# JeremyCJM/DiffSHEG

Measured on AMD Instinct MI355X. Metric: motion frames/sec (ddim25, n_poses=88), higher is better.
Workload: dtype bf16

## Files before the change

diffsheg_amd/_lib.py:

```python
from __future__ import annotations

import ctypes as C
import os

_HERE = os.path.dirname(os.path.abspath(__file__))
LIB_PATH = os.path.join(_HERE, "libdiffsheg_hip.so")


class DshError(RuntimeError):
    pass


class ModelConfigC(C.Structure):
    _fields_ = [("dim_pose", C.c_int32), ("expression_dim", C.c_int32), ("style_dim", C.c_int32),
                ("classifier_free", C.c_int32), ("cond_scale", C.c_float), ("latent_dim", C.c_int32),
                ("ff_size", C.c_int32), ("num_layers", C.c_int32), ("num_heads", C.c_int32),
                ("audio_dim", C.c_int32), ("aud_latent_dim", C.c_int32), ("hubert_dim", C.c_int32),
                ("hubert_enc_dim", C.c_int32), ("precision", C.c_int32), ("single_transformer", C.c_int32)]


class CrossAttnWeightsC(C.Structure):
    _fields_ = [(n, C.c_void_p) for n in ("norm_g", "norm_b", "text_norm_g", "text_norm_b", "wq", "bq", "wk", "bk", "wv", "bv",
                                           "sty_norm_g", "sty_norm_b", "sty_emb_w", "sty_emb_b", "sty_out_w", "sty_out_b")]

# ... 38 lines not shown
    "dsh_sample_num_steps_from": (C.c_int64, [C.POINTER(SamplerOptsC), C.c_int32, C.c_int32, C.c_int32]),
    "dsh_invert": (C.c_int, [_P, C.POINTER(SamplerOptsC), _P, C.c_int32, _P]),
    "dsh_invert_from": (C.c_int, [_P, C.POINTER(SamplerOptsC), _P, C.c_int32, C.c_int32, _P]),
    "dsh_set_guidance_scale": (C.c_int, [_P, C.POINTER(C.c_float), C.c_int32]),
    "dsh_diffusion_table": (C.c_int32, [C.c_int32, C.c_int32, C.c_char_p, C.POINTER(C.c_double), C.c_int32]),
    "dsh_timestep_map": (C.c_int32, [C.c_int32, C.c_int32, C.POINTER(C.c_int32), C.c_int32]),
    "dsh_jump_schedule": (C.c_int32, [C.c_int32, C.c_int32, C.c_int32, C.POINTER(C.c_int32), C.c_int32]),
    "dsh_interp_time": (C.c_int, [_P, _P, C.c_int32, C.c_int32, C.c_int32, _P, C.c_int32]),
    "dsh_interp_time_ragged": (C.c_int, [_P, _P, C.c_int32, C.c_int32, C.c_int32, _P, C.c_int32, _P, _P]),
    "dsh_inv_standardize": (C.c_int, [_P, _P, C.c_int64, C.c_int32, _P, _P, _P]),
    "dsh_axis_angle_to_euler": (C.c_int, [_P, _P, C.c_int64, C.c_int64, C.c_int32, _P, _P, _P, _P, _P, C.c_int64, _P, C.c_int64, _P, C.c_int32]),
    "dsh_euler_to_axis_angle": (C.c_int, [_P, _P, C.c_int64, C.c_int64, C.c_int32, _P, _P, _P, _P, _P, C.c_int64, _P, C.c_int32]),
    "dsh_op_gemm": (C.c_int, [_P, C.c_int32, _P, _P, _P, _P, _P, _P, C.c_int32, C.c_int32, C.c_int32, C.c_int32]),
    "dsh_op_gemm_f32_pro": (C.c_int, [_P, C.c_int32] + [_P, C.c_int32, C.c_int32] * 4 + [C.c_int32, _P, _P, _P, _P, C.c_int32, C.c_int32, C.c_int32, C.c_int32, _P, _P, C.c_int32, C.c_int32, C.c_int32, _P, C.c_int32, _P]),
    "dsh_debug_last_tl_variant": (C.c_int32, []),
    "dsh_debug_launch_counts": (C.c_int32, [C.POINTER(C.c_int64), C.c_int32, C.c_int32]),
    "dsh_op_tl_linear": (C.c_int, [_P, C.c_int32, _P, _P, _P, _P, _P, _P, C.c_int32, C.c_int32, C.c_int32, _P, _P, _P, C.c_int32, C.c_int32, C.c_int32]),
    "dsh_op_tl2_ffn": (C.c_int, [_P] * 12 + [C.c_int32, C.c_int32, _P, C.c_int32, _P, _P, C.c_int32]),
    "dsh_op_tl_aud_tail": (C.c_int, [_P] * 16 + [C.c_int32, C.c_int32, C.c_int32, _P, _P, C.c_int32]),
    "dsh_op_tl_aproj": (C.c_int, [_P, _P, _P, _P, C.c_int32, _P, _P, C.c_int32]),
    "dsh_op_tl_joint": (C.c_int, [_P, _P, C.c_int32, C.c_int32, C.c_int32, _P, _P, _P, C.c_int32, _P, C.c_int32, C.c_int32, _P]),
    "dsh_op_cross_attention": (C.c_int, [_P, C.POINTER(CrossAttnWeightsC), _P, _P, _P] + [C.c_int32] * 7 + [_P]),
    "dsh_op_linear_attention": (C.c_int, [_P, _P, C.c_int32, C.c_int32, C.c_int32, C.c_int32, _P]),
    "dsh_op_linear_attention_bf16": (C.c_int, [_P, _P, C.c_int32, C.c_int32, C.c_int32, C.c_int32, _P]),
    "dsh_op_linear_attention_ragged": (C.c_int, [_P, C.c_int32, C.c_int32, _P, C.c_int32, C.c_int32, C.c_int32, C.c_int32, _P, _P, C.c_int32, _P]),
    "dsh_op_linear_attention_tiled": (C.c_int, [_P, _P, C.c_int32, C.c_int32, C.c_int32, C.c_int32, _P, _P, C.c_int32, C.c_int32]),
    "dsh_op_layernorm": (C.c_int, [_P, _P, C.c_int32, C.c_int32, _P, _P, _P]),
    "dsh_op_ddim_step": (C.c_int, [_P] * 6 + [C.c_int32] * 3 + [C.c_float] * 4 + [C.c_int32] * 6),
    "dsh_op_philox_randn": (C.c_int, [_P, _P, C.c_int64, C.c_uint64, C.c_uint64]),
    "dsh_op_q_sample": (C.c_int, [_P] * 6 + [C.c_int32] * 6 + [C.c_uint64, C.c_uint64, C.POINTER(C.c_uint64), _P, C.POINTER(C.c_int32), C.c_uint64]),
# ... 101 lines not shown
```

diffsheg_amd/csrc/capi.hip:

```cpp
#include <algorithm>
#include <cmath>
#include <cstdio>
#include <cstdlib>
#include <cstring>
#include <map>
#include <memory>
#include <vector>

#include "../../include/diffsheg_hip.h"
#include "denoiser.h"
#include "audio_front.h"
#include "fgd.h"
#include "hubert.h"
#include "sampler.h"

namespace dsh {
static thread_local std::string g_last_error;
void set_last_error(const std::string& msg) { g_last_error = msg; }
const char* last_error_cstr() { return g_last_error.c_str(); }
}

struct dsh_ctx {
    dsh::ModelConfig cfg;
    hipStream_t stream = nullptr;
// ... 369 lines not shown
    dsh::GemmProArgs a{};
    a.pro = pro;
    a.seg[0] = x0; a.seg[1] = w1 ? x1 : nullptr; a.seg[2] = w2 ? x2 : nullptr; a.seg[3] = w3 ? x3 : nullptr;
    a.seg_ld[0] = ld0; a.seg_ld[1] = ld1; a.seg_ld[2] = ld2; a.seg_ld[3] = ld3;
    a.seg_end[0] = w0 / 32; a.seg_end[1] = a.seg_end[0] + w1 / 32; a.seg_end[2] = a.seg_end[1] + w2 / 32; a.seg_end[3] = a.seg_end[2] + w3 / 32;
    a.K = 32 * a.seg_end[3]; a.k_real = k_real;
    a.W = W; a.ldw = a.K; a.bias = bias; a.fc = fc;
    a.film = film; a.film_ld = film_ld; a.film_off = film_off; a.frames = frames; a.bmod = nb;
    a.R = R; a.ldr = N; a.C = C; a.ldc = N; a.M = M; a.N = N; a.act = act; a.nt_n = a.nt_m = 0;
    a.stats = stats; a.stat_groups = stat_groups; a.stat_gs = stat_groups > 0 ? a.K / stat_groups : 0; a.stats_out = stats_out;
    return dsh::launch_gemm_f32_pro(a, reinterpret_cast<hipStream_t>(hip_stream));
    API_END
}

int32_t dsh_debug_last_tl_variant(void) { return dsh::g_tl_last_variant; }

int32_t dsh_debug_launch_counts(int64_t* out, int32_t cap, int32_t reset) {
    for (int i = 0; i < dsh::LC_COUNT; ++i) {
        const long long v = reset ? dsh::g_launch_counts[i].exchange(0, std::memory_order_relaxed) : dsh::g_launch_counts[i].load(std::memory_order_relaxed);
        if (out && i < cap) out[i] = (int64_t)v;
    }
    return dsh::LC_COUNT;
}

namespace {
struct OpScratch {
    std::vector<void*> p;
    ~OpScratch() { for (void* q : p) (void)hipFree(q); }
    int alloc(void** out, size_t bytes) { DSH_HIP_CHECK(hipMalloc(out, bytes)); p.push_back(*out); return 0; }
    int upload(void** out, const void* host, size_t bytes) {
// ... 1180 lines not shown
```

diffsheg_amd/csrc/dsh_kernels.h:

```cpp
#pragma once
#include "dsh_common.h"

namespace dsh {

struct ConcatSegs {
    const float* p0; int ld0, w0;
    const void* p1;  int ld1, w1;
    const void* p2;  int ld2, w2;
    const float* p3; int ld3, w3;
};

struct GemmProArgs {
    int pro;
    const float* seg[4]; int seg_ld[4];
    int seg_end[4];
    int k_real;
    const float* W; int ldw;
    const float* bias;
    const float* fc;
    const float* film; int film_ld, film_off, frames, bmod;
    const float* R; int ldr;
    float* C; int ldc;
    int M, N, K, act;
    int nt_n, nt_m;
// ... 47 lines not shown
    int tls_nb0, tls_tb1;
    int dbg;
    unsigned long long* clk;
    unsigned long long* trace;
};
int launch_tl_linear(const TlArgs& a, int pro, hipStream_t s);
bool tl_linear_film_clips_ok(int frames, int bmod);
bool tls_linear_supported(const TlArgs& a, int pro);
bool tls_film_clips_ok(int frames, int bmod);
int launch_tls_linear(const TlArgs& a, int pro, hipStream_t s);
int tl_weight_src_row(int r);
int launch_tl_permute_weight(const void* W, int N, int K, void* dst, hipStream_t s);

int launch_tl2_linear(const TlArgs& a, int pro, hipStream_t s);
extern int g_tl_last_variant;
size_t tl2_frag_index(int K, int nt, int n, int k);
struct Tl2FfnArgs {
    const void* X;
    const void* Wffn;
    const float* b1; const float* b2; const float* b3;
    const float* film; int film_ld, film_off, frames, bmod, half_row0;
    const float* R; float* Cf; void* Ct;
    const float* row_const; int n_const_rows;
    int M;
    unsigned long long* trace;
    unsigned long long* clk;
    int stag_groups, stag_sleep;
    int rev;
    const void* Rhi; const void* Rlo; void* Clo;
};
// ... 112 lines not shown
```

diffsheg_amd/csrc/switches.h:

```cpp
#pragma once
#include <algorithm>
#include <atomic>
#include <cstdint>
#include <cstdlib>
#include <cstring>
#include <mutex>
#include <string>

namespace dsh {

enum SwitchKind : int { SWK_INT = 0, SWK_FLAG = 1, SWK_STR = 2 };
enum SwitchWhen : int { SWW_PROCESS = 0, SWW_CONTEXT = 1, SWW_CALL = 2 };
enum SwitchClass : int { SWC_PRODUCT = 0, SWC_AB_EXACT = 1, SWC_AB_ROUNDOFF = 2, SWC_BENCH = 3 };

#define DSH_SWITCH_TABLE(X)                                                                                                                      \
    X(DUAL, "DSH_DUAL", INT, "3", CONTEXT, PRODUCT, "most sub-batch streams of a large batch: 0 one stream, 1 two, n at most n (1 .. 8); results identical") \
    X(DUAL_LAG, "DSH_DUAL_LAG", INT, "3", CONTEXT, PRODUCT, "stream i + 1 starts this many token-per-lane launches behind stream i; the sampler reads it again per loop (CALL)") \
    X(DUAL_ROWS, "DSH_DUAL_ROWS", INT, "21500 (fp32: 2900)", CONTEXT, PRODUCT, "token rows per sub-batch stream; overrides only when positive") \
    X(DUAL_MIN_ROWS, "DSH_DUAL_MIN_ROWS", INT, "12288 (fp32: 4096)", CONTEXT, PRODUCT, "smallest batch (token rows) split over sub-batch streams; overrides only when positive") \
    X(PIPE, "DSH_PIPE", INT, "1", CALL, AB_EXACT, "sampling loops: the two encoders on two streams, the gesture encoder one step behind; 0 in sequence") \
    X(PIPE_ROWS, "DSH_PIPE_ROWS", INT, "64499", PROCESS, PRODUCT, "token rows below which a loop runs ONE batch with two encoder streams; latched in the sampler, read afresh (CONTEXT) by the sub-batch splitter") \
    X(NO_GRAPH, "DSH_NO_GRAPH", FLAG, "unset", CALL, PRODUCT, "present (any value, 0 included): small-batch evaluations are not replayed from a hipGraph") \
    X(GRAPH_ROWS, "DSH_GRAPH_ROWS", INT, "4096", PROCESS, PRODUCT, "token rows up to which a sampling loop replays its evaluations from a hipGraph") \
    X(LEVEL_CACHE, "DSH_LEVEL_CACHE", INT, "1", CALL, AB_EXACT, "x-independent part of an evaluation once per timestep level; 0 on every step") \
    X(LEVEL_PREFETCH, "DSH_LEVEL_PREFETCH", INT, "1", CALL, AB_EXACT, "that part ahead of the loop on a side stream; 0 inline at a level's first use") \
    X(TL2, "DSH_TL2", INT, "1", CONTEXT, AB_ROUNDOFF, "token-per-lane Linears: 0 first generation, 1 LDS-DMA kernels, 2 LDS-DMA everywhere (fp32 residual); dsh_op_tl_linear reads it per CALL") \
    X(TL2_ROLL, "DSH_TL2_ROLL", INT, "1", CALL, AB_EXACT, "rolling main loop of q|k|v / feat_proj.1 / ffn.linear2; 0 the round-2 loop") \
    X(TL2_ROT, "DSH_TL2_ROT", INT, "0", CALL, AB_EXACT, "rolling launches walk the weight tiles in a per-block rotated order (measured neutral)") \
    X(TL2_KSKIP, "DSH_TL2_KSKIP", INT, "1", CALL, AB_EXACT, "feat_proj.1 skips the trailing all-zero fragments of the concat row; 0 multiplies all 64") \
    X(TL2_HL, "DSH_TL2_HL", INT, "1", CONTEXT, AB_EXACT, "LDS-DMA kernels for the two residual-carrying Linears on hi / lo planes; 0 first generation") \
    X(FFN_FUSE, "DSH_FFN_FUSE", INT, "1", CONTEXT, AB_ROUNDOFF, "FFN branch as one fused launch; 0 three launches") \
    X(FFN_V, "DSH_FFN_V", INT, "3", CONTEXT, AB_ROUNDOFF, "fused FFN kernel generation: only 2 selects tl2_ffn_kernel, anything else tl3_ffn_kernel; dsh_op_tl2_ffn and the profiler's class text read it per CALL") \
    X(FFN_PC, "DSH_FFN_PC", INT, "1", CALL, AB_EXACT, "fused FFN phase C: 0 the round-4 loop, 1 pipelined across the phase boundary, 2 also pass-B epilogues early (clamped to 0 .. 2)") \
    X(FFN_PB, "DSH_FFN_PB", INT, "1", CALL, AB_EXACT, "fused FFN last stage (& 3): bit 0 hi plane kept in registers, bit 1 pass-B residual requested early; the denoiser's profiler byte count latches it") \
    X(FFN_X_IS_HI, "DSH_FFN_X_IS_HI", INT, "0", CALL, BENCH, "dsh_op_tl2_ffn on hi / lo planes: the input IS the hi plane of the residual, as in the denoiser's layers") \
    X(FFN_REPEAT, "DSH_FFN_REPEAT", INT, "0", CALL, BENCH, "dsh_op_tl2_ffn launches its kernel this many extra times (results unchanged)") \
    X(HILO, "DSH_HILO", INT, "1 (op entries: 0)", CONTEXT, AB_ROUNDOFF, "bf16 residual stream as hi + lo planes; 0 fp32 + bf16 shadow.  The op entries read it per CALL and take unset as OFF (hilo_denoiser / hilo_op below)") \
    X(TLS, "DSH_TLS", INT, "1", CONTEXT, AB_EXACT, "window-chain batches on the 32-token-block kernels of tl_small.hip; 0 off") \
    X(TLS_ROWS, "DSH_TLS_ROWS", INT, "per instantiation", CONTEXT, AB_EXACT, "token rows per launch up to which those kernels are used; overrides only when positive") \
    X(REV, "DSH_REV", INT, "1", CONTEXT, AB_EXACT, "alternate the row order of consecutive large token-per-lane launches; 0 off") \
    X(STAGGER, "DSH_STAGGER", STR, "unset", PROCESS, AB_EXACT, "\"groups,sleep[,mask]\" (%d,%d,%d): staggered first-round block start; mask bit 0 fused FFN, 1 q|k|v, 2 the other Linears") \
    X(SPLIT_AT, "DSH_SPLIT_AT", STR, "unset", PROCESS, BENCH, "\"c1,c2,...\": explicit sub-batch boundaries (clip indices); the list is latched, the once-only warning looks at its presence per CONTEXT") \
// ... 118 lines not shown
```

diffsheg_amd/csrc/tl2.hip:

```cpp
#include <algorithm>
#include <cstdio>
#include <cstdlib>
#include <type_traits>

#include "dsh_common.h"
#include "dsh_kernels.h"
#include "tl_common.h"
#include "switches.h"

namespace dsh {

namespace {

__device__ __forceinline__ void dma_sel(int k, const char* src_lane, char* lds_wave) {
    const char* s4 = src_lane + (k >> 2) * 4096;
    char* d4 = lds_wave + (k >> 2) * 4096;
    switch (k & 3) {
        case 0: __builtin_amdgcn_global_load_lds((gptr_t)s4, (lptr_t)d4, 16, 0, 0); break;
        case 1: __builtin_amdgcn_global_load_lds((gptr_t)s4, (lptr_t)d4, 16, 1024, 0); break;
        case 2: __builtin_amdgcn_global_load_lds((gptr_t)s4, (lptr_t)d4, 16, 2048, 0); break;
        default: __builtin_amdgcn_global_load_lds((gptr_t)s4, (lptr_t)d4, 16, 3072, 0); break;
    }
}
template <int N>
// ... 423 lines not shown
                    }
                }
                asm volatile("" : "+v"(prev));
            }
            if (PROBE) { pp.stamp(3); pp.roll(); }
        }
    };
    do_tile(nt0, std::true_type{});
    for (int nt = nt0 + 1; nt < nt1; ++nt) do_tile(nt, std::false_type{});
#pragma unroll
    for (int i = 0; i < NSTORE; ++i) store_piece(nt1 - 1, prev, i);
    trace_mark(p.trace, 2);
    if (PROBE) pp.dump(p.clk, pc0, pw0);
}

constexpr int FFN_MAXCLIP = 3;
constexpr int FFN_CH = 32 * 1024;
constexpr int FFN_LDS = 4 * FFN_CH + FFN_MAXCLIP * 4096 + (1024 + 3 * 512) * 4;
constexpr int FFN_NQ = 64 + 16;

template <bool PROBE>
__global__ __launch_bounds__(256, 1) void tl2_ffn_kernel(Tl2FfnArgs p) {
    extern __shared__ __attribute__((aligned(16))) char smem[];
    PhaseProbe pp;
    const unsigned long long pc0 = PROBE ? __builtin_readcyclecounter() : 0, pw0 = PROBE ? wall_clock64() : 0;
    trace_mark(p.trace, 0);
    start_stagger(p.stag_groups, p.stag_sleep);
    const int tid = threadIdx.x, lane = tid & 63;
    const int wave = __builtin_amdgcn_readfirstlane(tid >> 6);
    const int ml = lane & 31, h = lane >> 5;
// ... 297 lines not shown
        p.clk[(size_t)blockIdx.x * 8 + 7] = ((pc_ln - pc0) & 0xffffffffull) | ((__builtin_readcyclecounter() - pc0) << 32);
}

void tl_stagger_config(int which, int* groups, int* sleep) {
    struct Cfg { int g = 0, sl = 0, mask = 7; };
    static const Cfg cfg = [] {
        Cfg c;
        if (const char* e = switch_str(SW_STAGGER)) { int a = 0, b = 0, m = 7; const int n = sscanf(e, "%d,%d,%d", &a, &b, &m); if (n >= 2) { c.g = a; c.sl = b; if (n >= 3) c.mask = m; } }
        return c;
    }();
    const bool on = cfg.g > 1 && ((cfg.mask >> which) & 1);
    *groups = on ? cfg.g : 0; *sleep = on ? cfg.sl : 0;
}

int g_tl_last_variant = -1;

int launch_tl2_linear(const TlArgs& a, int pro, hipStream_t s) {
    DSH_REQUIRE(a.M > 0 && a.N > 0 && a.N % 32 == 0, "tl2_linear: N must be a positive multiple of 32");
    DSH_REQUIRE(a.K == 512 || a.K == 1024, "tl2_linear: K must be 512 or 1024");
    DSH_REQUIRE(a.ldx == (pro == 3 ? 512 : a.K), "tl2_linear: the tiled input must be exactly K features wide");
    DSH_REQUIRE(((uintptr_t)a.X % 16) == 0 && ((uintptr_t)a.W % 16) == 0, "tl2_linear: operands must be 16-byte aligned");
    DSH_REQUIRE(!a.Cf || !a.cf_rowmajor || a.ldcf % 4 == 0, "tl2_linear: row-major output leading dim");
    DSH_REQUIRE(!(a.cf_rowmajor && (a.R || a.Ct)), "tl2_linear: the row-major fp32 output has no residual / bf16 shadow");
    DSH_REQUIRE(pro >= 0 && pro <= 3, "tl2_linear: unknown prologue");
    const int tok = a.K == 512 ? 256 : 128;
    DSH_REQUIRE(pro != 1 && pro != 3 || (a.bias && a.row_const), "tl2_linear: folded LayerNorm needs d (bias) and c (row_const) vectors");
    DSH_REQUIRE(pro != 2 || (a.film && a.frames > 0 && a.bmod > 0 && a.film_ld % 4 == 0 && a.film_off % 4 == 0),
                "tl2_linear: FiLM prologue needs the folded film table");
    DSH_REQUIRE(pro != 2 || std::min((tok - 1) / a.frames + 2, a.bmod) <= T2_MAXCLIP,
                "tl2_linear: FiLM prologue: too many clips per 256-token block (clips shorter than 29 frames need batch <= 10)");
    DSH_REQUIRE(pro != 2 || a.K == 512, "tl2_linear: FiLM prologue is instantiated for K = 512");
    DSH_REQUIRE(!a.row_const || pro == 1 || pro == 3 || (pro == 2 && a.R && a.act == ACT_NONE),
                "tl2_linear: row_const is the CFG-null constant of the StylizationBlock instantiation or the c vector of a folded LayerNorm");
    DSH_REQUIRE(pro != 3 || (a.K == 1024 && a.X1 && a.X2 && a.kreal > 896 - 1 && a.kreal <= 1024), "tl2_linear: concat prologue arguments");
    const int mblocks = ceil_div(a.M, tok), ntiles = a.N / 32;
    int tpb = ntiles;
    if (mblocks < 128) { tpb = 1; while (tpb < ntiles && mblocks * ceil_div(ntiles, tpb) > 256) ++tpb; }
    TlArgs b = a;
    b.tiles_per_block = tpb;
    b.rot = switch_int(SW_TL2_ROT) != 0 ? 1 : 0;
    tl_stagger_config(pro == 1 ? 1 : 2, &b.stag_groups, &b.stag_sleep);
    if (mblocks < 256) { b.stag_groups = 0; b.stag_sleep = 0; }
    const dim3 grid(mblocks, ceil_div(ntiles, tpb)), block(a.K == 512 ? 512 : 256);
    const int lds = 4 * T2_CHUNK + 2 * a.N * 4;
    DSH_REQUIRE(lds <= 160 * 1024, "tl2_linear: N too large for the LDS bias table");
    typedef void (*kern_t)(TlArgs);
    struct Variant { int k, pro, has_r, out, act; kern_t fn; };
#define TLV(P, R, O, A) {512, P, R, O, A, tl2_linear_kernel<512, P, (R) != 0, O, A>}
#define TLV1K(P, R, O, A) {1024, P, R, O, A, tl2_linear_kernel<1024, P, (R) != 0, O, A>}
    static const Variant variants[] = {
        TLV(1, 0, 2, ACT_NONE),
        TLV(2, 1, 3, ACT_NONE),
        TLV(0, 0, 2, ACT_GELU),
        TLV(0, 0, 2, ACT_NONE), TLV(0, 1, 3, ACT_NONE), TLV(0, 0, 2, ACT_SILU), TLV(1, 0, 1, ACT_NONE),
        TLV(2, 0, 2, ACT_NONE), TLV(0, 1, 1, ACT_NONE), TLV(0, 0, 1, ACT_NONE),
        TLV(0, 0, 4, ACT_NONE),
        TLV1K(0, 0, 2, ACT_NONE),
        TLV1K(0, 0, 2, ACT_SILU),
// ... 14 lines not shown
    kern_t fn = nullptr;
    int variant = 0;
    for (int i = 0; i < NV; ++i)
        if (variants[i].k == a.K && variants[i].pro == pro && variants[i].has_r == has_r && variants[i].out == out && variants[i].act == a.act) fn = variants[i].fn;
    if (a.clk) {
        kern_t pf = nullptr;
        if (a.K == 512 && pro == 1 && !has_r && out == 2) pf = tl2_linear_kernel<512, 1, false, 2, ACT_NONE, true>;
        if (a.K == 512 && pro == 2 && has_r && out == 3) pf = tl2_linear_kernel<512, 2, true, 3, ACT_NONE, true>;
        if (a.K == 1024 && pro == 0 && !has_r && out == 2 && a.act == ACT_NONE) pf = tl2_linear_kernel<1024, 0, false, 2, ACT_NONE, true>;
        if (pf) {
            DSH_HIP_CHECK(hipFuncSetAttribute(reinterpret_cast<const void*>(pf), hipFuncAttributeMaxDynamicSharedMemorySize, 160 * 1024));
            fn = pf;
        } else b.clk = nullptr;
    }
    DSH_REQUIRE(fn != nullptr || a.Rlo, "tl2_linear: this (prologue, residual, outputs, activation) combination is not instantiated");
    const bool roll_on = switch_int(SW_TL2_ROLL) != 0;
    if (roll_on && !has_r && out == 2 && !b.clk && tpb == ntiles && ntiles >= 2) {
        kern_t rf = nullptr;
        if (a.K == 512 && pro == 1 && a.act == ACT_NONE) rf = tl2_linear_kernel<512, 1, false, 2, ACT_NONE, false, true>;
        else if (a.K == 1024 && pro == 3 && a.act == ACT_SILU) {
            const int nz = switch_int(SW_TL2_KSKIP) == 0 ? 0 : (1024 - round_up(a.kreal, 16)) / 16;
            rf = nz >= 8 ? (kern_t)tl2_linear_kernel<1024, 3, false, 2, ACT_SILU, false, true, false, 8>
               : nz >= 1 ? (kern_t)tl2_linear_kernel<1024, 3, false, 2, ACT_SILU, false, true, false, 1> : (kern_t)tl2_linear_kernel<1024, 3, false, 2, ACT_SILU, false, true>;
        }
        else if (a.K == 1024 && pro == 0 && a.act == ACT_NONE) rf = tl2_linear_kernel<1024, 0, false, 2, ACT_NONE, false, true>;
        if (rf) {
            static const bool rattr = [] {
                bool ok = true;
                auto set = [&](kern_t f) { ok &= hipFuncSetAttribute(reinterpret_cast<const void*>(f), hipFuncAttributeMaxDynamicSharedMemorySize, 160 * 1024) == hipSuccess; };
                set(tl2_linear_kernel<512, 1, false, 2, ACT_NONE, false, true>); set(tl2_linear_kernel<1024, 3, false, 2, ACT_SILU, false, true>);
                set(tl2_linear_kernel<1024, 3, false, 2, ACT_SILU, false, true, false, 8>); set(tl2_linear_kernel<1024, 3, false, 2, ACT_SILU, false, true, false, 1>);
                set(tl2_linear_kernel<1024, 0, false, 2, ACT_NONE, false, true>);
                return ok;
            }();
            DSH_REQUIRE(rattr, "tl2_linear: hipFuncSetAttribute failed for the rolling instantiations");
            fn = rf;
            variant = 1;
        }
    }
    if (a.Rlo) {
        DSH_REQUIRE(a.R && a.Clo && a.Ct && !a.Cf && a.act == ACT_NONE && ((a.K == 512 && pro == 2) || (a.K == 1024 && pro == 0)),
                    "tl2_linear: hi / lo residual planes are instantiated for the StylizationBlock (K = 512) and feat_proj.3 (K = 1024) launches");
        kern_t hf = a.K == 512 ? (kern_t)tl2_linear_kernel<512, 2, true, 3, ACT_NONE, false, true, true> : (kern_t)tl2_linear_kernel<1024, 0, true, 3, ACT_NONE, false, true, true>;
        static const bool hattr = [] {
            return hipFuncSetAttribute(reinterpret_cast<const void*>(tl2_linear_kernel<512, 2, true, 3, ACT_NONE, false, true, true>), hipFuncAttributeMaxDynamicSharedMemorySize, 160 * 1024) == hipSuccess &&
                   hipFuncSetAttribute(reinterpret_cast<const void*>(tl2_linear_kernel<1024, 0, true, 3, ACT_NONE, false, true, true>), hipFuncAttributeMaxDynamicSharedMemorySize, 160 * 1024) == hipSuccess;
        }();
        DSH_REQUIRE(hattr, "tl2_linear: hipFuncSetAttribute failed for the hi / lo instantiations");
        b.clk = nullptr;
        fn = hf;
        variant = 2;
    }
    g_tl_last_variant = variant;
    count_launch(variant == 1 ? LC_TL2_ROLL : variant == 2 ? LC_TL2_ROLL_HL : LC_TL2_LOOP);
    hipLaunchKernelGGL(fn, grid, block, lds, s, b);
    DSH_HIP_CHECK(hipGetLastError());
    return 0;
}

bool tl2_ffn_supported(int M, int frames, int bmod) {
    return M >= 128 * 64 && std::min((TL_TOK - 1) / frames + 2, bmod) <= FFN_MAXCLIP;
}

int launch_tl2_ffn(const Tl2FfnArgs& a, hipStream_t s) {
    DSH_REQUIRE(a.M > 0 && a.X && a.Wffn && a.b1 && a.b2 && a.b3 && a.film && a.R && a.Cf && a.Ct, "tl2_ffn: null operand");
    DSH_REQUIRE(a.frames > 0 && a.bmod > 0 && a.film_ld % 4 == 0 && a.film_off % 4 == 0, "tl2_ffn: folded FiLM table");
    DSH_REQUIRE(std::min((TL_TOK - 1) / a.frames + 2, a.bmod) <= FFN_MAXCLIP, "tl2_ffn: too many clips per 128-token block");
    static bool attr = false;
// ... 21 lines not shown
```

diffsheg_amd/csrc/tl_linear.hip:

```cpp
#include <algorithm>
#include <cstdlib>

#include "dsh_common.h"
#include "dsh_kernels.h"
#include "tl_common.h"

namespace dsh {

template <int KD, int PRO, bool HAS_R, int OUT, int ACT, int ABL = 0, bool HL = false>
__global__ __launch_bounds__(256, (KD == 512 ? 2 : 1)) void tl_linear_kernel(TlArgs p) {
    static_assert(!HL || (HAS_R && OUT == 3 && ACT == ACT_NONE && ABL == 0), "hi / lo planes: the residual-carrying instantiations only");
    constexpr int TL_K = KD, NFRAG = KD / 16, NST = KD / TL_STAGE_K;
    constexpr bool HAS_C = (PRO == 2 && HAS_R && ACT == ACT_NONE);
    constexpr int LDS_W = tl_lds_bytes(KD);
    extern __shared__ __attribute__((aligned(16))) char smem[];
    const int tid = threadIdx.x, lane = tid & 63, wave = tid >> 6;
    unsigned long long clk0 = 0, rt0 = 0;
    if (p.clk) { clk0 = __builtin_readcyclecounter(); rt0 = wall_clock64(); }
    const int ml = lane & 31, h = lane >> 5;
    const int bx = tl_block_index(p.rev);
    const int tb = bx * (TL_TOK / 32) + wave;
    const int row = tb * 32 + ml;
    const int lane_off = ml * 32 + h * 16;

// ... 254 lines not shown
                }
            }
        }
    }
    if (p.clk && blockIdx.x == 0 && blockIdx.y == 0 && tid == 0) {
        p.clk[0] = __builtin_readcyclecounter() - clk0;
        p.clk[1] = wall_clock64() - rt0;
        p.clk[2] = bar_cyc;
    }
}

bool tl_linear_film_clips_ok(int frames, int bmod) { return frames > 0 && bmod > 0 && std::min((TL_TOK - 1) / frames + 2, bmod) <= TL_MAXCLIP; }

int launch_tl_linear(const TlArgs& a, int pro, hipStream_t s) {
    g_tl_last_variant = 10;
    DSH_REQUIRE(a.M > 0 && a.N > 0 && a.N % 32 == 0, "tl_linear: N must be a positive multiple of 32");
    DSH_REQUIRE(a.K == 512 || a.K == 1024, "tl_linear: K must be 512 or 1024");
    DSH_REQUIRE(a.ldx == (pro == 3 ? 512 : a.K), "tl_linear: the tiled input must be exactly K features wide");
    DSH_REQUIRE(((uintptr_t)a.X % 16) == 0 && ((uintptr_t)a.W % 16) == 0, "tl_linear: operands must be 16-byte aligned");
    DSH_REQUIRE(!a.Cf || !a.cf_rowmajor || a.ldcf % 4 == 0, "tl_linear: row-major output leading dim");
    DSH_REQUIRE(!(a.cf_rowmajor && (a.R || a.Ct)), "tl_linear: the row-major fp32 output has no residual / bf16 shadow");
    DSH_REQUIRE(pro == 0 || (a.gamma && a.beta), "tl_linear: LayerNorm prologue needs gamma/beta");
    DSH_REQUIRE(pro != 2 || (a.film && a.frames > 0 && a.bmod > 0 && a.film_ld % 4 == 0 && a.film_off % 4 == 0),
                "tl_linear: FiLM prologue needs the folded film table");
    DSH_REQUIRE(pro != 2 || tl_linear_film_clips_ok(a.frames, a.bmod),
                "tl_linear: FiLM prologue: too many clips per 128-token block (clips shorter than 26 frames need batch <= 6)");
    DSH_REQUIRE(pro != 2 || a.K == 512, "tl_linear: FiLM prologue is instantiated for K = 512");
    const int mblocks = ceil_div(a.M, TL_TOK), ntiles = a.N / 32, slots = a.K == 512 ? 512 : 256;
    int tpb = ntiles;
    if (mblocks < 256) { tpb = 1; while (tpb < ntiles && mblocks * ceil_div(ntiles, tpb) > slots) ++tpb; }
// ... 76 lines not shown
```

diffsheg_amd/csrc/tl_small.hip:

```cpp
#include "dsh_kernels.h"
#include "tl_common.h"

#include <algorithm>
#include <cstdlib>

namespace dsh {
namespace {

__device__ __forceinline__ void mfma16_lds_b(f32x16& acc, const u32x4* a, const char* lds_lane) {
    u32x4 bw[2][4];
#pragma unroll
    for (int i = 0; i < 4; ++i) bw[0][i] = *reinterpret_cast<const u32x4*>(lds_lane + i * 1024);
#pragma unroll
    for (int g = 0; g < 4; ++g) {
        if (g + 1 < 4) {
#pragma unroll
            for (int i = 0; i < 4; ++i) bw[(g + 1) & 1][i] = *reinterpret_cast<const u32x4*>(lds_lane + ((g + 1) * 4 + i) * 1024);
        }
#pragma unroll
        for (int i = 0; i < 4; ++i)
            acc = __builtin_amdgcn_mfma_f32_32x32x16_bf16(__builtin_bit_cast(bf16x8, a[g * 4 + i]), __builtin_bit_cast(bf16x8, bw[g & 1][i]), acc, 0, 0, 0);
    }
}

// ... 215 lines not shown
bool tls_film_clips_ok(int frames, int bmod) { return frames > 0 && bmod > 0 && std::min(31 / frames + 2, bmod) <= TLS_MAXCLIP; }

bool tls_linear_supported(const TlArgs& a, int pro) {
    if (a.M <= 0 || a.N <= 0 || a.N % 128 != 0 || !a.bias || !a.X || !a.W) return false;
    if (a.frames <= 0 || a.bmod <= 0) return false;
    const int Mc = a.frames * a.bmod;
    if (a.M != Mc && !(a.M > Mc && (a.M - Mc) % 32 == 0 && a.M - Mc >= Mc)) return false;
    if ((pro == 1 || pro == 3) && !a.row_const) return false;
    if (pro == 2 && !(a.film && a.film_ld % 4 == 0 && a.film_off % 4 == 0 && tls_film_clips_ok(a.frames, a.bmod))) return false;
    if (pro == 3 && !(a.X1 && a.X2 && a.kreal > 896 - 1 && a.kreal <= 1024)) return false;
    return tls_pick(a, pro) != nullptr;
}

int launch_tls_linear(const TlArgs& a, int pro, hipStream_t s) {
    g_tl_last_variant = 11;
    DSH_REQUIRE(tls_linear_supported(a, pro), "tls_linear: this launch is not covered by the window-chain kernels");
    DSH_REQUIRE(((uintptr_t)a.X % 16) == 0 && ((uintptr_t)a.W % 16) == 0, "tls_linear: operands must be 16-byte aligned");
    tls_kern_t fn = tls_pick(a, pro);
    static bool attr = false;
    if (!attr) {
        const tls_kern_t all[] = {tls_linear_kernel<512, 2, true, ACT_NONE>, tls_linear_kernel<1024, 0, true, ACT_NONE>,
                                  tls_linear_kernel<512, 1, false, ACT_NONE>, tls_linear_kernel<512, 0, false, ACT_GELU>,
                                  tls_linear_kernel<1024, 0, false, ACT_NONE>, tls_linear_kernel<1024, 3, false, ACT_SILU>};
        for (tls_kern_t k : all)
            DSH_HIP_CHECK(hipFuncSetAttribute(reinterpret_cast<const void*>(k), hipFuncAttributeMaxDynamicSharedMemorySize, 64 * 1024));
        attr = true;
    }
    TlArgs b = a;
    const int Mc = a.frames * a.bmod, nbh = ceil_div(std::min(a.M, Mc), 32);
    b.tls_nb0 = nbh;
// ... 11 lines not shown
```

include/diffsheg_hip.h:

```cpp
#ifndef DIFFSHEG_HIP_H
#define DIFFSHEG_HIP_H

#include <stdint.h>

#ifdef __cplusplus
extern "C" {
#endif

typedef struct dsh_ctx dsh_ctx;

enum { DSH_PRECISION_FP32 = 0, DSH_PRECISION_BF16 = 1 };
enum { DSH_SAMPLER_DDIM = 0, DSH_SAMPLER_DDPM = 1 };
enum { DSH_NOISE_STACK = 0, DSH_NOISE_PHILOX = 1 };

typedef struct dsh_model_config {
    int32_t dim_pose;
    int32_t expression_dim;
    int32_t style_dim;
    int32_t classifier_free;
    float   cond_scale;
    int32_t latent_dim;
    int32_t ff_size;
    int32_t num_layers;
    int32_t num_heads;
// ... 75 lines not shown
                        float* y);
int dsh_axis_angle_to_euler(void* hip_stream, const float* x, int64_t ld_x, int64_t rows, int32_t joints, const float* mean_aa,
                            const float* std_aa, const float* mean_e, const float* std_e, float* y_std, int64_t ld_std, float* y_deg,
                            int64_t ld_deg, const int32_t* lengths_dev, int32_t frames);
int dsh_euler_to_axis_angle(void* hip_stream, const float* x, int64_t ld_x, int64_t rows, int32_t joints, const float* mean_e,
                            const float* std_e, const float* mean_aa, const float* std_aa, float* y, int64_t ld_y,
                            const int32_t* lengths_dev, int32_t frames);

int dsh_op_gemm(void* hip_stream, int32_t dtype, const void* A, const void* W, const float* bias, const float* R,
                float* Cf, void* Ct, int32_t M, int32_t N, int32_t K, int32_t act);
int dsh_op_gemm_f32_pro(void* hip_stream, int32_t pro, const float* x0, int32_t ld0, int32_t w0, const float* x1, int32_t ld1, int32_t w1,
                        const float* x2, int32_t ld2, int32_t w2, const float* x3, int32_t ld3, int32_t w3, int32_t k_real, const float* W,
                        const float* bias, const float* fc, const float* film, int32_t film_ld, int32_t film_off, int32_t frames, int32_t nb,
                        const float* R, float* C, int32_t M, int32_t N, int32_t act, const float* stats, int32_t stat_groups, float* stats_out);
int32_t dsh_debug_last_tl_variant(void);
#define DSH_LAUNCH_COUNT_ENTRIES 17
int32_t dsh_debug_launch_counts(int64_t* out, int32_t cap, int32_t reset);
int dsh_op_tl_linear(void* hip_stream, int32_t pro, const void* X, const void* W, const float* bias, const float* R,
                     float* Cf, void* Ct, int32_t M, int32_t N, int32_t act, const float* gamma, const float* beta,
                     const float* film, int32_t frames, int32_t nb, int32_t K);
int dsh_op_tl2_ffn(void* hip_stream, const void* X, const float* Hres, const void* W1, const float* b1, const void* W2, const float* b2,
                   const void* W3, const float* b3, const float* gamma, const float* beta, const float* film, int32_t frames, int32_t nb,
                   const float* row_const, int32_t n_const_rows, float* Cf, void* Ct, int32_t M);
int dsh_op_tl_aud_tail(void* hip_stream, const void* Y, const float* X2, const float* ws1, const float* bs1, const float* w1, const float* b1,
                       const float* w2, const float* b2, const float* ws2, const float* bs2, const float* g1, const float* be1, const float* g2,
                       const float* be2, const float* film, int32_t frames, int32_t nb, int32_t Mc, float* out_f, void* out_b, int32_t ld_b);
int dsh_op_tl_aproj(void* hip_stream, const void* X, const float* W, const float* bias, int32_t n_enc, void* out0, void* out1, int32_t Mc);
int dsh_op_tl_joint(void* hip_stream, const float* x, int32_t ldx, int32_t c0, int32_t w, const float* Wj, const float* bias, const float* pe,
                    int32_t frames, const float* cnull, int32_t Mc, int32_t row1, float* h_out);
typedef struct dsh_cross_attn_weights {
// ... 142 lines not shown
```

Before: 157,900.

## Run q|k|v projection on 4 waves of 64 tokens each

Adds a dedicated q|k|v rolling kernel in which each wave holds two 32-token row blocks, one in VGPRs and one in AGPRs. Each LDS weight fragment then feeds two MFMAs, and the block uses 256 threads instead of 512. The aim is to halve LDS weight reads and DMA traffic per token and to interleave epilogue work for both blocks inside the MFMA stream. In exchange, register pressure is very high and fewer waves are resident for latency hiding. The new kernel becomes the default for K=512 rolling launches, and setting the roll switch to 2 restores the old path.

```diff
diff --git a/diffsheg_amd/_lib.py b/diffsheg_amd/_lib.py
--- a/diffsheg_amd/_lib.py
+++ b/diffsheg_amd/_lib.py
@@ -76,6 +76,7 @@
     "dsh_op_gemm": (C.c_int, [_P, C.c_int32, _P, _P, _P, _P, _P, _P, C.c_int32, C.c_int32, C.c_int32, C.c_int32]),
     "dsh_op_gemm_f32_pro": (C.c_int, [_P, C.c_int32] + [_P, C.c_int32, C.c_int32] * 4 + [C.c_int32, _P, _P, _P, _P, C.c_int32, C.c_int32, C.c_int32, C.c_int32, _P, _P, C.c_int32, C.c_int32, C.c_int32, _P, C.c_int32, _P]),
     "dsh_debug_last_tl_variant": (C.c_int32, []),
+    "dsh_debug_last_tl_wave_tokens": (C.c_int32, []),
     "dsh_debug_launch_counts": (C.c_int32, [C.POINTER(C.c_int64), C.c_int32, C.c_int32]),
     "dsh_op_tl_linear": (C.c_int, [_P, C.c_int32, _P, _P, _P, _P, _P, _P, C.c_int32, C.c_int32, C.c_int32, _P, _P, _P, C.c_int32, C.c_int32, C.c_int32]),
     "dsh_op_tl2_ffn": (C.c_int, [_P] * 12 + [C.c_int32, C.c_int32, _P, C.c_int32, _P, _P, C.c_int32]),
diff --git a/diffsheg_amd/csrc/capi.hip b/diffsheg_amd/csrc/capi.hip
--- a/diffsheg_amd/csrc/capi.hip
+++ b/diffsheg_amd/csrc/capi.hip
@@ -407,6 +407,7 @@
 }
 
 int32_t dsh_debug_last_tl_variant(void) { return dsh::g_tl_last_variant; }
+int32_t dsh_debug_last_tl_wave_tokens(void) { return dsh::g_tl_last_wave_tokens; }
 
 int32_t dsh_debug_launch_counts(int64_t* out, int32_t cap, int32_t reset) {
     for (int i = 0; i < dsh::LC_COUNT; ++i) {
diff --git a/diffsheg_amd/csrc/dsh_kernels.h b/diffsheg_amd/csrc/dsh_kernels.h
--- a/diffsheg_amd/csrc/dsh_kernels.h
+++ b/diffsheg_amd/csrc/dsh_kernels.h
@@ -85,6 +85,7 @@
 
 int launch_tl2_linear(const TlArgs& a, int pro, hipStream_t s);
 extern int g_tl_last_variant;
+extern int g_tl_last_wave_tokens;
 size_t tl2_frag_index(int K, int nt, int n, int k);
 struct Tl2FfnArgs {
     const void* X;
diff --git a/diffsheg_amd/csrc/switches.h b/diffsheg_amd/csrc/switches.h
--- a/diffsheg_amd/csrc/switches.h
+++ b/diffsheg_amd/csrc/switches.h
@@ -25,7 +25,7 @@
     X(LEVEL_CACHE, "DSH_LEVEL_CACHE", INT, "1", CALL, AB_EXACT, "x-independent part of an evaluation once per timestep level; 0 on every step") \
     X(LEVEL_PREFETCH, "DSH_LEVEL_PREFETCH", INT, "1", CALL, AB_EXACT, "that part ahead of the loop on a side stream; 0 inline at a level's first use") \
     X(TL2, "DSH_TL2", INT, "1", CONTEXT, AB_ROUNDOFF, "token-per-lane Linears: 0 first generation, 1 LDS-DMA kernels, 2 LDS-DMA everywhere (fp32 residual); dsh_op_tl_linear reads it per CALL") \
-    X(TL2_ROLL, "DSH_TL2_ROLL", INT, "1", CALL, AB_EXACT, "rolling main loop of q|k|v / feat_proj.1 / ffn.linear2; 0 the round-2 loop") \
+    X(TL2_ROLL, "DSH_TL2_ROLL", INT, "1", CALL, AB_EXACT, "rolling main loop of q|k|v / feat_proj.1 / ffn.linear2, q|k|v on 4 waves of 64 tokens; 2 q|k|v on 8 waves of 32 as the others; 0 the round-2 loop") \
     X(TL2_ROT, "DSH_TL2_ROT", INT, "0", CALL, AB_EXACT, "rolling launches walk the weight tiles in a per-block rotated order (measured neutral)") \
     X(TL2_KSKIP, "DSH_TL2_KSKIP", INT, "1", CALL, AB_EXACT, "feat_proj.1 skips the trailing all-zero fragments of the concat row; 0 multiplies all 64") \
     X(TL2_HL, "DSH_TL2_HL", INT, "1", CONTEXT, AB_EXACT, "LDS-DMA kernels for the two residual-carrying Linears on hi / lo planes; 0 first generation") \
diff --git a/diffsheg_amd/csrc/tl2.hip b/diffsheg_amd/csrc/tl2.hip
--- a/diffsheg_amd/csrc/tl2.hip
+++ b/diffsheg_amd/csrc/tl2.hip
@@ -461,6 +461,173 @@
     if (PROBE) pp.dump(p.clk, pc0, pw0);
 }
 
+__global__ __attribute__((amdgpu_flat_work_group_size(256, 256), amdgpu_waves_per_eu(1, 1)))
+void tl2_qkv_w64_kernel(TlArgs p) {
+    constexpr int NW = 4, NTHR = NW * 64, ND = 32 / NW, NFRAG = 32;
+    extern __shared__ __attribute__((aligned(16))) char smem[];
+    trace_mark(p.trace, 0);
+    start_stagger(p.stag_groups, p.stag_sleep);
+    const int tid = threadIdx.x, lane = tid & 63;
+    const int wave = __builtin_amdgcn_readfirstlane(tid >> 6);
+    const int ml = lane & 31, h = lane >> 5;
+    const int bx = tl_block_index(p.rev);
+    const int tb0 = bx * (2 * NW) + 2 * wave;
+    const int lane_off = ml * 32 + h * 16;
+    const int NT = p.N / 32;
+    const int nt0 = blockIdx.y * p.tiles_per_block;
+    const int nt1 = (nt0 + p.tiles_per_block) < NT ? (nt0 + p.tiles_per_block) : NT;
+    const int p0 = nt0, p1 = nt1;
+    char* wdst = smem + wave * (ND * 1024);
+    const __amdgpu_buffer_rsrc_t wrsrc = __builtin_amdgcn_make_buffer_rsrc(const_cast<void*>(p.W), 0, p.N * 512 * 2, 0x00020000);
+    const int wvoff = wave * (ND * 1024) + lane * 16;
+    const int ntl = nt1 - nt0;
+    const int rot = p.rot ? (int)((unsigned)(bx >> 3) % (unsigned)ntl) : 0;
+    auto ptile = [&](int nt) -> int { const int t = nt + rot; return t >= nt1 ? t - ntl : t; };
+    auto dma_soff = [&](int q) -> int { return ptile(q < p1 ? q : p1 - 1) * T2_CHUNK; };
+    auto dma_dst = [&](int q) -> char* { return wdst + (q & 3) * T2_CHUNK; };
+    auto issue_chunk = [&](int q) {
+#pragma unroll
+        for (int k = 0; k < ND; ++k) dma_buf(k, wrsrc, wvoff, dma_soff(q), dma_dst(q));
+    };
+    issue_chunk(p0);
+    issue_chunk(p0 + 1);
+    u32x4 fragA[NFRAG], fragB[NFRAG];
+    {
+        const char* xr = reinterpret_cast<const char*>(p.X) + (size_t)tb0 * NFRAG * 1024 + lane_off;
+#pragma unroll
+        for (int s = 0; s < NFRAG; ++s) fragA[s] = *reinterpret_cast<const u32x4*>(xr + s * 1024);
+#pragma unroll
+        for (int s = 0; s < NFRAG; ++s) fragB[s] = *reinterpret_cast<const u32x4*>(xr + (NFRAG + s) * 1024);
+    }
+    float* sbias = reinterpret_cast<float*>(smem + 4 * T2_CHUNK);
+    float* sconst = sbias + p.N;
+    for (int i = tid; i < p.N; i += NTHR) {
+        sbias[i] = p.bias[i];
+        sconst[i] = p.row_const[i];
+    }
+    float rstd[2], nmr[2];
+    {
+        float sum, sq;
+        row_moments_bf16<NFRAG>(fragA, sum, sq);
+        float mean = sum / 512.f;
+        sq = fmaxf(sq - sum * mean, 0.f);
+        rstd[0] = 1.0f / sqrtf(sq / 512.f + 1e-5f);
+        nmr[0] = -mean * rstd[0];
+        row_moments_bf16<NFRAG>(fragB, sum, sq);
+        mean = sum / 512.f;
+        sq = fmaxf(sq - sum * mean, 0.f);
+        rstd[1] = 1.0f / sqrtf(sq / 512.f + 1e-5f);
+        nmr[1] = -mean * rstd[1];
+    }
+#pragma unroll
+    for (int s = 0; s < NFRAG; ++s) {
+        asm volatile("" ::"v"(fragA[s]));
+        asm volatile("" : "+a"(fragB[s]));
+    }
+    asm volatile("s_waitcnt vmcnt(0)" ::: "memory");
+    __syncthreads();
+    issue_chunk(p0 + 2);
+    trace_mark(p.trace, 1);
+
+    char* Ctb = reinterpret_cast<char*>(p.Ct);
+    typedef __attribute__((address_space(3))) const char* lcptr_t;
+    typedef __attribute__((address_space(3))) const u32x4* lfrag_t;
+    const char* lds_lane_r = smem + lane * 16;
+    auto chunk_base = [&](int q) -> lcptr_t { lcptr_t b = (lcptr_t)lds_lane_r + (q & 3) * T2_CHUNK; asm volatile("" : "+v"(b)); return b; };
+    u32x4 aw[2][4];
+    f32x16 acc0A, acc0B, acc1A, acc1B;
+    constexpr int VMW = ND + 7;
+    auto mid_barrier = [&]() {
+        asm volatile("s_waitcnt vmcnt(%0)\n\ts_waitcnt lgkmcnt(0)" ::"n"(VMW) : "memory");
+        __builtin_amdgcn_s_barrier();
+        asm volatile("" ::: "memory");
+        __builtin_amdgcn_sched_barrier(0);
+    };
+    auto slot_reads = [&](int m, lcptr_t cur, lcptr_t nxt) {
+        auto rd = [&](int f) { aw[(f >> 2) & 1][f & 3] = *(lfrag_t)(cur + f * 1024); };
+        if (m < 24) rd(m + 4);
+        if (m >= 20 && m < 24) rd(m + 8);
+        if (m >= 28) aw[0][m - 28] = *(lfrag_t)(nxt + (m - 28) * 1024);
+    };
+    struct Epi { float v[8]; u32x4 o[2]; };
+    f32x4 d4, c4;
+    auto epi_step = [&](int ts, int nte, const f32x16& E, Epi& st, int qi, int step, auto inloop_tag) {
+        constexpr bool INLOOP = decltype(inloop_tag)::value;
+        if (step == 0) {
+            if (ts == 0) {
+                const int col = nte * 32 + 16 * (qi >> 1) + 8 * h + 4 * (qi & 1);
+                d4 = *reinterpret_cast<const f32x4*>(sbias + col);
+                c4 = *reinterpret_cast<const f32x4*>(sconst + col);
+            }
+        } else if (step <= 4) {
+            const int e = step - 1;
+            float x = E[4 * qi + e];
+            if constexpr (INLOOP) { const float ev = x; asm volatile("v_accvgpr_read_b32 %0, %1" : "=v"(x) : "a"(ev)); }
+            x = fmaf(x, rstd[ts], fmaf(nmr[ts], c4[e], d4[e]));
+            asm volatile("" : "+v"(x));
+            st.v[4 * (qi & 1) + e] = x;
+        } else if (step == 5) {
+            u32x4 o;
+            o.x = pack_bf16(st.v[0], st.v[1]); o.y = pack_bf16(st.v[2], st.v[3]);
+            o.z = pack_bf16(st.v[4], st.v[5]); o.w = pack_bf16(st.v[6], st.v[7]);
+            asm volatile("" : "+v"(o));
+            st.o[qi >> 1] = o;
+        } else {
+            const u32x4 o = st.o[qi >> 1];
+            u32x4* dst = reinterpret_cast<u32x4*>(Ctb + ((size_t)(tb0 + ts) * (2 * NT) + 2 * nte + (qi >> 1)) * 1024 + lane_off);
+            __builtin_nontemporal_store(o, dst);
+        }
+    };
+    auto epi_slot = [&](int ts, int nte, const f32x16& E, Epi& st, auto m_tag, auto inloop_tag) {
+        constexpr int m = decltype(m_tag)::value;
+        if constexpr (m == 1 || m == 7 || m == 13 || m == 19) epi_step(ts, nte, E, st, (m - 1) / 6, 0, inloop_tag);
+        if constexpr (m >= 3 && m <= 24 && (m - 3) % 6 < 4) epi_step(ts, nte, E, st, (m - 3) / 6, 1 + (m - 3) % 6, inloop_tag);
+        if constexpr (m == 13 || m == 25) epi_step(ts, nte, E, st, m == 13 ? 1 : 3, 5, inloop_tag);
+        if constexpr (m == 28 || m == 29) epi_step(ts, nte, E, st, m == 28 ? 1 : 3, 6, inloop_tag);
+    };
+    auto tile = [&](int nt, f32x16& W0, f32x16& W1, const f32x16& E0, const f32x16& E1, auto prev_tag) {
+        constexpr bool HAS_PREV = decltype(prev_tag)::value;
+        Epi st0, st1;
+        const int pprev = HAS_PREV ? ptile(nt - 1) : 0;
+        const lcptr_t cur = chunk_base(nt), nxt = chunk_base(nt + 1);
+        const int so_next = dma_soff(nt + 3);
+        char* dst_next = dma_dst(nt + 3);
+        static_for<32>([&](auto m_tag) {
+            constexpr int m = decltype(m_tag)::value;
+            const f32x16 z = {0.f, 0.f, 0.f, 0.f, 0.f, 0.f, 0.f, 0.f, 0.f, 0.f, 0.f, 0.f, 0.f, 0.f, 0.f, 0.f};
+            const bf16x8 a = __builtin_bit_cast(bf16x8, aw[(m >> 2) & 1][m & 3]);
+            W0 = __builtin_amdgcn_mfma_f32_32x32x16_bf16(a, __builtin_bit_cast(bf16x8, fragA[m]), m == 0 ? z : W0, 0, 0, 0);
+            if ((m & 3) == 1) dma_buf(m >> 2, wrsrc, wvoff, so_next, dst_next);
+            if (HAS_PREV) epi_slot(0, pprev, E0, st0, m_tag, std::true_type{});
+            __builtin_amdgcn_sched_barrier(0);
+            W1 = __builtin_amdgcn_mfma_f32_32x32x16_bf16(a, __builtin_bit_cast(bf16x8, fragB[m]), m == 0 ? z : W1, 0, 0, 0);
+            slot_reads(m, cur, nxt);
+            if (HAS_PREV) epi_slot(1, pprev, E1, st1, m_tag, std::true_type{});
+            __builtin_amdgcn_sched_barrier(0);
+            if (m == 27) mid_barrier();
+        });
+    };
+#pragma unroll
+    for (int i = 0; i < 4; ++i) aw[0][i] = *reinterpret_cast<const u32x4*>(lds_lane_r + (p0 & 3) * T2_CHUNK + i * 1024);
+    __builtin_amdgcn_sched_barrier(0);
+    tile(nt0, acc0A, acc1A, acc0B, acc1B, std::false_type{});
+    int nt = nt0 + 1;
+    for (; nt + 1 < nt1; nt += 2) {
+        tile(nt, acc0B, acc1B, acc0A, acc1A, std::true_type{});
+        tile(nt + 1, acc0A, acc1A, acc0B, acc1B, std::true_type{});
+    }
+    Epi st0, st1;
+    if (nt < nt1) {
+        tile(nt, acc0B, acc1B, acc0A, acc1A, std::true_type{});
+        const int pl = ptile(nt);
+        static_for<32>([&](auto m2) { epi_slot(0, pl, acc0B, st0, m2, std::false_type{}); epi_slot(1, pl, acc1B, st1, m2, std::false_type{}); });
+    } else {
+        const int pl = ptile(nt1 - 1);
+        static_for<32>([&](auto m2) { epi_slot(0, pl, acc0A, st0, m2, std::false_type{}); epi_slot(1, pl, acc1A, st1, m2, std::false_type{}); });
+    }
+    trace_mark(p.trace, 2);
+}
+
 constexpr int FFN_MAXCLIP = 3;
 constexpr int FFN_CH = 32 * 1024;
 constexpr int FFN_LDS = 4 * FFN_CH + FFN_MAXCLIP * 4096 + (1024 + 3 * 512) * 4;
@@ -788,6 +955,7 @@
 }
 
 int g_tl_last_variant = -1;
+int g_tl_last_wave_tokens = 0;
 
 int launch_tl2_linear(const TlArgs& a, int pro, hipStream_t s) {
     DSH_REQUIRE(a.M > 0 && a.N > 0 && a.N % 32 == 0, "tl2_linear: N must be a positive multiple of 32");
@@ -815,7 +983,9 @@
     b.rot = switch_int(SW_TL2_ROT) != 0 ? 1 : 0;
     tl_stagger_config(pro == 1 ? 1 : 2, &b.stag_groups, &b.stag_sleep);
     if (mblocks < 256) { b.stag_groups = 0; b.stag_sleep = 0; }
-    const dim3 grid(mblocks, ceil_div(ntiles, tpb)), block(a.K == 512 ? 512 : 256);
+    const dim3 grid(mblocks, ceil_div(ntiles, tpb));
+    dim3 block(a.K == 512 ? 512 : 256);
+    int wave_tokens = 32;
     const int lds = 4 * T2_CHUNK + 2 * a.N * 4;
     DSH_REQUIRE(lds <= 160 * 1024, "tl2_linear: N too large for the LDS bias table");
     typedef void (*kern_t)(TlArgs);
@@ -860,7 +1030,8 @@
         } else b.clk = nullptr;
     }
     DSH_REQUIRE(fn != nullptr || a.Rlo, "tl2_linear: this (prologue, residual, outputs, activation) combination is not instantiated");
-    const bool roll_on = switch_int(SW_TL2_ROLL) != 0;
+    const long roll = switch_int(SW_TL2_ROLL);
+    const bool roll_on = roll != 0;
     if (roll_on && !has_r && out == 2 && !b.clk && tpb == ntiles && ntiles >= 2) {
         kern_t rf = nullptr;
         if (a.K == 512 && pro == 1 && a.act == ACT_NONE) rf = tl2_linear_kernel<512, 1, false, 2, ACT_NONE, false, true>;
@@ -882,6 +1053,13 @@
             DSH_REQUIRE(rattr, "tl2_linear: hipFuncSetAttribute failed for the rolling instantiations");
             fn = rf;
             variant = 1;
+            if (a.K == 512 && roll != 2) {
+                static const bool wattr = hipFuncSetAttribute(reinterpret_cast<const void*>(tl2_qkv_w64_kernel), hipFuncAttributeMaxDynamicSharedMemorySize, 160 * 1024) == hipSuccess;
+                DSH_REQUIRE(wattr, "tl2_linear: hipFuncSetAttribute failed for the 64-token-per-wave q|k|v kernel");
+                fn = tl2_qkv_w64_kernel;
+                block = dim3(256);
+                wave_tokens = 64;
+            }
         }
     }
     if (a.Rlo) {
@@ -898,6 +1076,7 @@
         variant = 2;
     }
     g_tl_last_variant = variant;
+    g_tl_last_wave_tokens = wave_tokens;
     count_launch(variant == 1 ? LC_TL2_ROLL : variant == 2 ? LC_TL2_ROLL_HL : LC_TL2_LOOP);
     hipLaunchKernelGGL(fn, grid, block, lds, s, b);
     DSH_HIP_CHECK(hipGetLastError());
diff --git a/diffsheg_amd/csrc/tl_linear.hip b/diffsheg_amd/csrc/tl_linear.hip
--- a/diffsheg_amd/csrc/tl_linear.hip
+++ b/diffsheg_amd/csrc/tl_linear.hip
@@ -292,6 +292,7 @@
 
 int launch_tl_linear(const TlArgs& a, int pro, hipStream_t s) {
     g_tl_last_variant = 10;
+    g_tl_last_wave_tokens = 32;
     DSH_REQUIRE(a.M > 0 && a.N > 0 && a.N % 32 == 0, "tl_linear: N must be a positive multiple of 32");
     DSH_REQUIRE(a.K == 512 || a.K == 1024, "tl_linear: K must be 512 or 1024");
     DSH_REQUIRE(a.ldx == (pro == 3 ? 512 : a.K), "tl_linear: the tiled input must be exactly K features wide");
diff --git a/diffsheg_amd/csrc/tl_small.hip b/diffsheg_amd/csrc/tl_small.hip
--- a/diffsheg_amd/csrc/tl_small.hip
+++ b/diffsheg_amd/csrc/tl_small.hip
@@ -253,6 +253,7 @@
 
 int launch_tls_linear(const TlArgs& a, int pro, hipStream_t s) {
     g_tl_last_variant = 11;
+    g_tl_last_wave_tokens = 32;
     DSH_REQUIRE(tls_linear_supported(a, pro), "tls_linear: this launch is not covered by the window-chain kernels");
     DSH_REQUIRE(((uintptr_t)a.X % 16) == 0 && ((uintptr_t)a.W % 16) == 0, "tls_linear: operands must be 16-byte aligned");
     tls_kern_t fn = tls_pick(a, pro);
diff --git a/include/diffsheg_hip.h b/include/diffsheg_hip.h
--- a/include/diffsheg_hip.h
+++ b/include/diffsheg_hip.h
@@ -113,6 +113,7 @@
                         const float* bias, const float* fc, const float* film, int32_t film_ld, int32_t film_off, int32_t frames, int32_t nb,
                         const float* R, float* C, int32_t M, int32_t N, int32_t act, const float* stats, int32_t stat_groups, float* stats_out);
 int32_t dsh_debug_last_tl_variant(void);
+int32_t dsh_debug_last_tl_wave_tokens(void);
 #define DSH_LAUNCH_COUNT_ENTRIES 17
 int32_t dsh_debug_launch_counts(int64_t* out, int32_t cap, int32_t reset);
 int dsh_op_tl_linear(void* hip_stream, int32_t pro, const void* X, const void* W, const float* bias, const float* R,
```

New measurement: 158,600 (median of 6 runs). No clear change (+0.4%).
